# lmdu/pyfastx

Hardware: AMD Instinct MI355X
Metric: FASTA index build + 1M random 100bp subseq fetches, 3 Gbp plain FASTA per GPU (throughput of the whole step, stream resident in HBM) (higher is better)
Workload: dtype u8; 1 GPU; configs[1]: synthetic 3.0 Gbp hg38-shaped plain FASTA per GPU (200 contigs, 60-col LF, soft-masked, N runs), index build + 1000000 random 100 bp intervals (50% '-' strand); parallelism=one GPU, the whole stream resident in its HBM

## Files before the change

### pyfastx_amd/csrc/fx_kernels.hpp

```cpp
#pragma once
#include <hip/hip_runtime.h>
#include <stdint.h>

namespace fx {

constexpr int BLOCK = 256;
constexpr int UNROLL = 8;
constexpr int CHUNK = 16;
constexpr int TILE = BLOCK * CHUNK * UNROLL;

__device__ __forceinline__ uint32_t zero_bytes(uint32_t x) {
    return ~(((x & 0x7F7F7F7Fu) + 0x7F7F7F7Fu) | x | 0x7F7F7F7Fu);
}
__device__ __forceinline__ uint32_t flags4(uint32_t t) { return __builtin_amdgcn_udot4(t, 0x08040201u, 0u, false) >> 7; }
__device__ __forceinline__ uint32_t eq_mask16(const uint4 &v, uint32_t pat) {
    uint32_t lo = __builtin_amdgcn_udot4(zero_bytes(v.x ^ pat), 0x08040201u, 0u, false);
    lo = __builtin_amdgcn_udot4(zero_bytes(v.y ^ pat), 0x80402010u, lo, false);
    uint32_t hi = __builtin_amdgcn_udot4(zero_bytes(v.z ^ pat), 0x08040201u, 0u, false);
    hi = __builtin_amdgcn_udot4(zero_bytes(v.w ^ pat), 0x80402010u, hi, false);
    return (lo >> 7) | (hi << 1);
}

__device__ __forceinline__ uint4 load16(const uint8_t *__restrict__ data, int64_t p, int64_t n) {
    if (p + CHUNK <= n) return *reinterpret_cast<const uint4 *>(data + p);
// ... 337 lines not shown
            }
            rank += total;
        }
        if (ok) {
            int64_t got = rank - skip;
            got = got < 0 ? 0 : (got > take ? take : got);
            if ((fl & 2) && got < take && got > 0) {
                const int64_t delta = take - got;
                for (int64_t j0 = 0; j0 < got; j0 += G) {
                    const int64_t j = j0 + sub;
                    uint8_t c = 0;
                    if (j < got) c = out[delta + j];
                    if (j < got) out[j] = c;
                }
            }
            if (sub == 0 && q.out_len) q.out_len[i] = got;
        }
    }
}

template <int G, int NP, bool COAL = false>
__global__ __launch_bounds__(BLOCK) void k_fetch_lines(const uint8_t *__restrict__ data, int64_t gbase, int64_t n_bytes, FetchQ q, FastaTab tab,
                                                      int64_t nq, int flags_all, uint8_t *__restrict__ dst, int32_t *__restrict__ list,
                                                      int *__restrict__ list_n) {
    __shared__ uint8_t lut[256];
    constexpr int CO_CAP = 2048;
    __shared__ __attribute__((aligned(16))) uint32_t s_out[COAL ? BLOCK / 64 : 1][COAL ? (CO_CAP + 32) / 4 : 1];
    constexpr int TABCAP = 512;
    __shared__ int64_t s_boff[TABCAP], s_slen[TABCAP];
    __shared__ int32_t s_llen[TABCAP], s_en[TABCAP];
    const int64_t n_seq = tab.n_seq_dev ? (*tab.n_seq_dev < tab.n_seq ? (int64_t)*tab.n_seq_dev : tab.n_seq) : tab.n_seq;
    const bool tab_lds = n_seq <= TABCAP && n_seq > 0;
    build_comp_lut(lut);
    if (tab_lds)
        for (int r = threadIdx.x; r < (int)n_seq; r += BLOCK) {
            s_boff[r] = tab.boff[r]; s_slen[r] = tab.slen[r];
            const int64_t ll = tab.llen[r];
            s_llen[r] = ll > 0x7FFFFFFFll ? 0x7FFFFFFF : (int32_t)ll;
            s_en[r] = tab.elen[r] | (tab.norm[r] << 8);
        }
    __syncthreads();
    constexpr int QPW = 64 / G;
    const int lane = lane_id(), sub = lane & (G - 1), grp = lane / G;
    const int64_t wave = ((int64_t)blockIdx.x * BLOCK + threadIdx.x) >> 6;
    const int64_t nwaves = ((int64_t)gridDim.x * BLOCK) >> 6;
    int64_t d_id = 0, d_a = 0, d_b = 0, d_off = 0;
    int d_fl = flags_all;
    auto fetch_desc = [&](int64_t i) {
// ... 349 lines not shown
```

### pyfastx_amd/csrc/fx_spanscan.hpp

```cpp
#pragma once
#include "fx_kernels.hpp"

namespace fx {

#ifndef FX_GRAN
#define FX_GRAN 4096
#endif
constexpr int GRAN = FX_GRAN;
constexpr int GR_ROWS = GRAN / (64 * CHUNK);
constexpr int SPAN_GRANS = 65536 / GRAN;
constexpr int SPAN = GRAN * SPAN_GRANS;
constexpr uint32_t SP_NONE = 0xFFFFFFFFu;

struct GranOut { uint32_t n, h, first, last, v1, c1, v2, c2, ovf; };
struct __attribute__((aligned(16))) GranPk { uint32_t nh, fl, d1, d2; };
__device__ __forceinline__ GranPk gran_pack(const GranOut &o) {
    GranPk p;
    p.nh = o.n | (o.h << 16); p.fl = (o.first & 0xFFFFu) | (o.last << 16);
    p.d1 = o.v1 | (o.c1 << 16); p.d2 = o.v2 | (o.c2 << 16) | (o.ovf << 31);
    return p;
}
__device__ __forceinline__ GranOut gran_unpack(const GranPk &p) {
    GranOut o;
    o.n = p.nh & 0xFFFFu; o.h = p.nh >> 16;
// ... 206 lines not shown
    }
    const int64_t g0 = (((int64_t)blockIdx.x * blockDim.x + threadIdx.x) >> 6) * SCAN_GPW;
    uint4 v[SCAN_GPW][GR_ROWS];
#pragma unroll
    for (int k = 0; k < SCAN_GPW; ++k) if (g0 + k < g_end) granule_load<true>(v[k], data, n, is_last, g0 + k);
    uint32_t L = 0, hmask = 0;
#pragma unroll
    for (int k = 0; k < SCAN_GPW; ++k)
        if (g0 + k < g_end && granule_body<MODE>(v[k], data, prev_byte, g0 + k, out, L)) hmask |= 1u << k;
    if (MODE == 0 && lane_id() == 0) {
#pragma unroll
        for (int k = 0; k < SCAN_GPW; ++k) if ((hmask >> k) & 1u) hl_g[atomicAdd(&hl_n, 1u)] = (uint32_t)(g0 + k);
        __threadfence_block();
        if (atomicAdd(&hl_done, 1u) == (blockDim.x >> 6) - 1) {
            const uint32_t cnt = hl_n;
            if (cnt) {
                const uint32_t base = atomicAdd(hgl.count, cnt);
                for (uint32_t k = 0; k < cnt; ++k) hgl.g[base + k] = hl_g[k];
            }
        }
    }
}

constexpr int CHUNK_GRANS = 1024;
struct ChunkTot { long long n, h, last, pad; };
struct Totals {
    long long n_nl, n_hdr, last_nl, seq_len, pad0, pad1, pad2, pad3;
};

__device__ __forceinline__ long long shfl_up64(long long v, int d) {
    const int lo = __shfl_up((int)(v & 0xFFFFFFFFll), d, 64), hi = __shfl_up((int)(v >> 32), d, 64);
    return ((long long)hi << 32) | (unsigned int)lo;
}
__device__ __forceinline__ long long shfl64(long long v, int l) {
    const int lo = __shfl((int)(v & 0xFFFFFFFFll), l, 64), hi = __shfl((int)(v >> 32), l, 64);
    return ((long long)hi << 32) | (unsigned int)lo;
}
struct Tri { long long n, h, last; };
__device__ __forceinline__ Tri tri_join(const Tri &a, const Tri &b) { return Tri{a.n + b.n, a.h + b.h, a.last > b.last ? a.last : b.last}; }
__device__ __forceinline__ Tri tri_wave_incl(Tri v) {
    const int l = lane_id();
#pragma unroll
    for (int d = 1; d < 64; d <<= 1) {
        const Tri t{shfl_up64(v.n, d), shfl_up64(v.h, d), shfl_up64(v.last, d)};
        if (l >= d) v = tri_join(t, v);
    }
    return v;
}
__device__ __forceinline__ Tri tri_block_incl(Tri v, Tri *lds, Tri *total) {
    const int w = threadIdx.x >> 6, l = lane_id(), nw = (blockDim.x + 63) >> 6;
    const Tri inc = tri_wave_incl(v);
    __syncthreads();
    if (l == 63) lds[w] = inc;
    __syncthreads();
    Tri base{0, 0, -1}, tot{0, 0, -1};
    for (int i = 0; i < nw; ++i) { const Tri s = lds[i]; if (i < w) base = tri_join(base, s); tot = tri_join(tot, s); }
    *total = tot;
    return tri_join(base, inc);
}
__device__ __forceinline__ Tri gran_tri(const GranPk *__restrict__ go, int64_t g, int64_t ngran, int64_t gbase) {
    if (g >= ngran) return Tri{0, 0, -1};
    const GranOut o = gran_unpack(go[g]);
    return Tri{(long long)o.n, (long long)o.h, o.n ? gbase + g * (long long)GRAN + o.last : -1};
}

template <int MODE, int CG>
__global__ __launch_bounds__(CG) void k_gran_reduce(const uint8_t *__restrict__ data, int64_t n, int prev_byte,
                                                   int is_last, GranList hgl, GranPk *__restrict__ go,
                                                   int64_t ngran, int64_t gbase, ChunkTot *__restrict__ ct) {
    __shared__ Tri lds[CG / 64];
    if (blockIdx.x == gridDim.x - 1) {
        if (threadIdx.x < 64) {
            uint32_t L = 0;
            const uint32_t h_w = granule<false, MODE>(data, n, prev_byte, is_last, ngran - 1, go, L);
            if (MODE == 0 && h_w && threadIdx.x == 0) hgl.g[atomicAdd(hgl.count, 1u)] = (uint32_t)(ngran - 1);
        }
        __threadfence_block();
        __syncthreads();
    }
    Tri tot;
    tri_block_incl(gran_tri(go, (int64_t)blockIdx.x * CG + threadIdx.x, ngran, gbase), lds, &tot);
    if (threadIdx.x == 0) ct[blockIdx.x] = ChunkTot{tot.n, tot.h, tot.last, 0};
}

struct Tri32 { uint32_t n, h; int32_t last; };
__device__ __forceinline__ Tri32 tri32_block_incl(Tri32 v, uint32_t (*lds)[16], Tri32 *total) {
    const int w = threadIdx.x >> 6, l = lane_id(), nw = (blockDim.x + 63) >> 6;
#pragma unroll
    for (int d = 1; d < 64; d <<= 1) {
        const uint32_t a = __shfl_up(v.n, d, 64), b = __shfl_up(v.h, d, 64);
        const int32_t c = __shfl_up(v.last, d, 64);
        if (l >= d) { v.n += a; v.h += b; v.last = c > v.last ? c : v.last; }
    }
// ... 370 lines not shown
    const int64_t cnt = *irr.count;
    int64_t i = wave, g = i < cnt ? irr.g[i] : 0;
    uint4 v[GR_ROWS];
    if (i < cnt) {
#pragma unroll
        for (int j = 0; j < GR_ROWS; ++j) v[j] = load16(x.data, g * (int64_t)GRAN + j * 1024 + lane * CHUNK, x.n);
    }
    for (; i < cnt; i += nwaves) {
        const int64_t gc = g, hb = x.hdr_prefix[gc];
        int64_t he = x.hdr_prefix[gc + 1];
        if (he > cap) he = cap;
        ExactMasks mk;
        exact_masks(x, v, is_last, prev_byte, gc, he > hb, mk);
        if (i + nwaves < cnt) {
            g = irr.g[i + nwaves];
#pragma unroll
            for (int j = 0; j < GR_ROWS; ++j) v[j] = load16(x.data, g * (int64_t)GRAN + j * 1024 + lane * CHUNK, x.n);
        }
        exact_rows(x, rv, cap, gc, hb, mk);
    }
}

__global__ __launch_bounds__(BLOCK) void k_fasta_finalize2(int64_t cap, FastaCols c, Totals *__restrict__ tot,
                                                          const uint8_t *__restrict__ data, int64_t n_bytes, int64_t gbase) {
    const int64_t *__restrict__ hdr = c.hoff, *__restrict__ hdr_line = c.hdr_line;
    const int64_t k = (int64_t)blockIdx.x * BLOCK + threadIdx.x;
    const int64_t n_hdr = tot->n_hdr < cap ? tot->n_hdr : cap;
    int64_t s = 0;
    if (k < n_hdr) {
        if (c.dlen[k] >= 0) {
            int64_t hn, Ln;
            if (k + 1 < n_hdr) { hn = hdr[k + 1]; Ln = hdr_line[k + 1]; }
            else               { hn = tot->last_nl + 1; Ln = tot->n_nl; }
            const int64_t nseq = Ln - hdr_line[k] - 1;
            const int64_t blen = hn - c.boff[k];
            s = blen - (int64_t)c.elen[k] * nseq;
            c.blen[k] = blen; c.slen[k] = s;
            const int norm = c.bad[k] > 1 ? 0 : 1;
            c.norm[k] = norm;
            int reg = line_regular(data, n_bytes, gbase, c.boff[k], blen, s, nseq > 0 ? c.llen[k] : 0, c.elen[k], norm);
            if (reg < 0) reg = c.bad[k] == 0;
            c.reg[k] = reg;
        } else { c.blen[k] = 0; c.slen[k] = 0; c.norm[k] = 1; c.reg[k] = 0; }
    }
    __shared__ unsigned long long blk;
    if (threadIdx.x == 0) blk = 0;
    __syncthreads();
    s = wave_sum64(s);
    if (lane_id() == 0 && s) atomicAdd(&blk, (unsigned long long)s);
    __syncthreads();
    if (threadIdx.x == 0 && blk) atomicAdd((unsigned long long *)&tot->seq_len, blk);
}

__global__ __launch_bounds__(BLOCK) void k_line_regular(const uint8_t *__restrict__ data, int64_t n_bytes, int64_t gbase, int64_t n,
                                                       const int64_t *__restrict__ boff, const int64_t *__restrict__ blen,
                                                       const int64_t *__restrict__ slen, const int64_t *__restrict__ llen,
                                                       const int32_t *__restrict__ elen, const int32_t *__restrict__ norm,
                                                       int32_t *__restrict__ reg) {
    const int64_t k = (int64_t)blockIdx.x * BLOCK + threadIdx.x;
    if (k < n) reg[k] = line_regular(data, n_bytes, gbase, boff[k], blen[k], slen[k], llen[k], elen[k], norm[k]) > 0 ? 1 : 0;
}

__device__ __forceinline__ int64_t prev_nl_wave(const ScanCtx &x, int64_t p) {
    const int64_t y = (p - x.gbase < x.n) ? p - x.gbase : x.n;
    if (y <= 0) return -1;
    const int64_t g = (y - 1) / GRAN;
    const int64_t a = g * (int64_t)GRAN + lane_id() * 64;
    unsigned long long m = 0;
#pragma unroll
    for (int i = 0; i < 4; ++i)
        if (a + i * CHUNK < y) m |= (unsigned long long)eq_mask16(load16(x.data, a + i * CHUNK, x.n), 0x0A0A0A0Au) << (16 * i);
    if (y - a < 64) m &= (y - a <= 0) ? 0ull : (~0ull >> (64 - (y - a)));
    const unsigned long long b = __ballot(m != 0);
    if (!b) return x.prevnl[g];
// ... 220 lines not shown
```

### pyfastx_amd/csrc/fxgpu.hip

```cpp
#include <hip/hip_runtime.h>
#include <zlib.h>
#include <fcntl.h>
#include <pthread.h>
#include <sched.h>
#include <sys/mman.h>
#include <sys/stat.h>
#include <unistd.h>

#include <algorithm>
#include <atomic>
#include <chrono>
#include <functional>
#include <map>
#include <memory>
#include <cstdarg>
#include <cstdio>
#include <cstdlib>
#include <cstring>
#include <mutex>
#include <string>
#include <thread>
#include <vector>

#include "../../include/fxgpu.h"
// ... 307 lines not shown
static void stage_drop(fx_handle *h);
struct fx_handle {
    int device = 0;
    hipStream_t stream = nullptr;
    StageAsync *stage = nullptr;
    int stage_fd = -1;
    hipStream_t stream2 = nullptr;
    uint8_t *d_data = nullptr;
    uint8_t *d_alloc = nullptr;
    size_t blob_cap = 0;
    bool owns = false;
    int64_t n = 0;
    bool gz = false;
    int64_t base = 0;
    int prev_byte = '\n';
    bool is_last = true;
    int64_t n_nl = 0;
    bool scanned = false;
    int64_t ngran = 0;
    DevBuf<GranPk> gran;
    DevBuf<uint32_t> hdr_grans, irr_grans;
    DevBuf<ChunkTot> chunks;
    DevBuf<unsigned long long> ctl;
    Totals *pin_tot = nullptr;
    struct OneBox { int64_t off, blen, skip, take, dst_off, out_len; } *one_box = nullptr;
    uint8_t *one_out = nullptr;
    Mailbox *mb = nullptr;
    hipStream_t mb_stream = nullptr;
    unsigned long long mb_seq = 0;
    bool mb_running = false, mb_off = false;
    DevBuf<uint32_t> nm_table;
    DevBuf<int64_t> nm_off;
    uint64_t nm_mask = 0;
    int nm_kind = -1;
    DevBuf<int64_t> nl_prefix, hdr_prefix, prevnl;
    DevBuf<int64_t> hdr, fa_boff, fa_blen, fa_slen, fa_llen, fa_hdr_line;
    DevBuf<int32_t> fa_elen, fa_norm, fa_dlen, fa_name_len, fa_reg;
    DevBuf<uint32_t> fa_bad;
    int64_t n_hdr = 0, fa_seqlen = 0;
    bool fasta_built = false;
    bool build_pending = false;
    int pending_full_name = 0;
    DevBuf<uint32_t> comp_runs;
    int comp_gpw = 0;
    bool comp_runs_valid = false;
    DevBuf<int64_t> fq_name_off, fq_rlen, fq_soff, fq_qoff;
// ... 1538 lines not shown
static ScanCtx scan_ctx(const fx_handle *h) {
    ScanCtx x;
    x.data = h->d_data; x.n = h->n; x.gbase = h->base; x.ngran = h->ngran;
    x.go = h->gran.p; x.nl_prefix = h->nl_prefix.p; x.hdr_prefix = h->hdr_prefix.p; x.prevnl = h->prevnl.p;
    return x;
}
static FastaCols fasta_cols(fx_handle *h) {
    FastaCols c;
    c.hoff = h->hdr.p; c.boff = h->fa_boff.p; c.blen = h->fa_blen.p; c.slen = h->fa_slen.p; c.llen = h->fa_llen.p;
    c.hdr_line = h->fa_hdr_line.p; c.elen = h->fa_elen.p; c.dlen = h->fa_dlen.p; c.name_len = h->fa_name_len.p;
    c.norm = h->fa_norm.p; c.bad = h->fa_bad.p; c.reg = h->fa_reg.p;
    return c;
}
static int alloc_fasta_table(fx_handle *h, int64_t cap) {
    int rc;
    if ((rc = h->hdr.alloc(cap)) || (rc = h->fa_hdr_line.alloc(cap)) || (rc = h->fa_boff.alloc(cap)) ||
        (rc = h->fa_blen.alloc(cap)) || (rc = h->fa_slen.alloc(cap)) || (rc = h->fa_llen.alloc(cap)) ||
        (rc = h->fa_elen.alloc(cap)) || (rc = h->fa_norm.alloc(cap)) || (rc = h->fa_dlen.alloc(cap)) ||
        (rc = h->fa_name_len.alloc(cap)) || (rc = h->fa_bad.alloc(cap)) || (rc = h->fa_reg.alloc(cap)))
        return rc;
    return FX_OK;
}

static Totals *ctl_totals(fx_handle *h) { return (Totals *)h->ctl.p; }
static uint32_t *ctl_counter(fx_handle *h, int i) { return (uint32_t *)(h->ctl.p + 8 + i); }

static int comp_run_granules(int64_t ngran) {
    return ngran >= 65536 ? 4 * COMP_DEPTH : ngran >= 16384 ? 2 * COMP_DEPTH : COMP_DEPTH;
}

template <int MODE>
static int granule_pass(fx_handle *h, bool fq_lines = false, bool with_comp = false) {
    int rc;
    const int64_t nfull = h->n / GRAN, ngran = nfull + 1;
    const bool small = ngran <= (2ll << 20);
    const int64_t cg = small ? 256 : 1024, nchunks = (ngran + cg - 1) / cg;
    h->ngran = ngran;
    if ((rc = h->gran.alloc(ngran)) || (rc = h->hdr_grans.alloc(ngran)) || (MODE == 0 && (rc = h->irr_grans.alloc(ngran))) ||
        (rc = h->chunks.alloc(nchunks)) ||
        (rc = h->ctl.alloc(64)) || (rc = h->nl_prefix.alloc(ngran + 1)) || (rc = h->hdr_prefix.alloc(ngran + 1)) ||
        (rc = h->prevnl.alloc(ngran + 1)))
        return rc;
    if (!h->pin_tot) HIPCHK(hipHostMalloc((void **)&h->pin_tot, sizeof(Totals), hipHostMallocDefault));
    HIPCHK(hipMemsetAsync(h->ctl.p, 0, 64 * sizeof(unsigned long long), h->stream));
    GranList hgl{h->hdr_grans.p, ctl_counter(h, 0)};
    const int SCAN_WG = 512;
    if (nfull > 0 && MODE == 1 && fq_lines) {
        if ((rc = h->fq_lines.alloc((nfull + FQR_G - 1) / FQR_G * FQR_G * FQL_CAP))) return rc;
        if (with_comp) {
            const int64_t nruns = (nfull + FQLC_G - 1) / FQLC_G;
            if ((rc = h->fq_runs.alloc(nruns)) || (rc = h->fq_acc_build.alloc(1)) || (rc = h->fq_rej.alloc(nruns + 1))) return rc;
            static const int64_t grid_cap = [] { const char *e = getenv("FX_FQ_FUSED_GRID"); return e && atoll(e) > 0 ? atoll(e) : 6144ll; }();
            static const int force_crlf = [] { const char *e = getenv("FX_FQ_CRLF"); return e ? atoi(e) : -1; }();
            if (force_crlf >= 0 ? force_crlf != 0 : h->fq_crlf)
                FX_LAUNCH(h, K_FASTQ_LINES, k_fastq_lines_comp<true>, dim3((unsigned)std::min<int64_t>(nblocks(nruns, BLOCK / 64), grid_cap)), dim3(BLOCK), h->d_data,
                          h->n, h->prev_byte, nfull, h->gran.p, h->fq_lines.p, hgl, h->fq_runs.p, nruns);
            else
                FX_LAUNCH(h, K_FASTQ_LINES, k_fastq_lines_comp<false>, dim3((unsigned)std::min<int64_t>(nblocks(nruns, BLOCK / 64), grid_cap)), dim3(BLOCK), h->d_data,
                          h->n, h->prev_byte, nfull, h->gran.p, h->fq_lines.p, hgl, h->fq_runs.p, nruns);
        } else
        FX_LAUNCH(h, K_FASTQ_LINES, k_fastq_lines, dim3(nblocks(nfull, (BLOCK / 64) * FQL_G)), dim3(BLOCK), h->d_data, h->n, h->prev_byte, nfull,
                  h->gran.p, h->fq_lines.p, hgl);
    } else if (nfull > 0 && MODE == 0 && with_comp) {
        const int gpw = comp_run_granules(ngran);
        const int64_t runs = (ngran + gpw - 1) / gpw;
        if ((rc = h->comp_runs.alloc(runs * RUN_WORDS))) return rc;
        HIPCHK(hipMemsetAsync(h->comp_runs.p, 0, (size_t)runs * RUN_WORDS * 4, h->stream));
        FX_LAUNCH(h, K_SCAN_COMP, k_scan_comp, dim3(nblocks(runs, COMP_WPB)), dim3(COMP_WPB * 64), h->d_data, h->n, h->prev_byte,
                  (int)h->is_last, nfull, h->gran.p, hgl, gpw, h->comp_runs.p);
        h->comp_gpw = gpw;
        h->comp_runs_valid = true;
    } else if (nfull > 0)
        FX_LAUNCH(h, K_SPAN_SCAN, (k_span_scan<MODE>), dim3(nblocks((nfull + SCAN_GPW - 1) / SCAN_GPW * 64, SCAN_WG)), dim3(SCAN_WG), h->d_data, h->n,
                  h->prev_byte, (int)h->is_last, nfull, h->gran.p, hgl);
    if (small) {
        FX_LAUNCH(h, K_GRAN_REDUCE, (k_gran_reduce<MODE, 256>), dim3((unsigned)nchunks), dim3(256), h->d_data, h->n, h->prev_byte,
                  (int)h->is_last, hgl, h->gran.p, ngran, h->base, h->chunks.p);
        FX_LAUNCH(h, K_GRAN_PREFIX, (k_gran_prefix<256>), dim3((unsigned)nchunks), dim3(256), h->gran.p, ngran, h->base,
                  h->chunks.p, ctl_totals(h), h->nl_prefix.p, h->hdr_prefix.p, h->prevnl.p);
    } else {
        FX_LAUNCH(h, K_GRAN_REDUCE, (k_gran_reduce<MODE, 1024>), dim3((unsigned)nchunks), dim3(1024), h->d_data, h->n, h->prev_byte,
                  (int)h->is_last, hgl, h->gran.p, ngran, h->base, h->chunks.p);
        FX_LAUNCH(h, K_GRAN_PREFIX, (k_gran_prefix<1024>), dim3((unsigned)nchunks), dim3(1024), h->gran.p, ngran, h->base,
                  h->chunks.p, ctl_totals(h), h->nl_prefix.p, h->hdr_prefix.p, h->prevnl.p);
    }
    if (MODE == 1 && fq_lines && with_comp && nfull > 0) {
        FastqAcc init;
        memset(&init, 0, sizeof init);
        init.minqs = 104; init.maxqs = 33;
        HIPCHK(hipMemcpyAsync(h->fq_acc_build.p, &init, sizeof init, hipMemcpyHostToDevice, h->stream));
        const int64_t nruns = (nfull + FQLC_G - 1) / FQLC_G;
        HIPCHK(hipMemsetAsync(h->fq_rej.p, 0, 4, h->stream));
        FX_LAUNCH(h, K_FASTQ_COMP, k_fastq_comp_reduce, dim3((unsigned)std::min<int64_t>(nblocks(nruns, BLOCK), 1024)), dim3(BLOCK), (const FqRun *)h->fq_runs.p,
                  nruns, (const int64_t *)h->nl_prefix.p, (int64_t)0, h->d_data, h->n, nfull, h->fq_acc_build.p, h->fq_rej.p);
    }
    HIPCHK(hipGetLastError());
    return FX_OK;
}

static int enqueue_records(fx_handle *h, int full_name) {
    const ScanCtx x = scan_ctx(h);
    const int64_t cap = h->hdr.cap, ngran = h->ngran;
    const FastaCols c = fasta_cols(h);
    const RecView rv{h->fa_boff.p, h->fa_llen.p, h->fa_dlen.p, h->fa_bad.p, h->hdr.p};
    const GranList hgl{h->hdr_grans.p, ctl_counter(h, 0)}, irr{h->irr_grans.p, ctl_counter(h, 1)};
    FX_LAUNCH(h, K_HDR_REC, k_hdr_rec, dim3(2048), dim3(BLOCK), x, h->prev_byte, (int)h->is_last, full_name, hgl, c, cap);
    FX_LAUNCH(h, K_GRAN_LINES, k_gran_lines, dim3(nblocks(ngran, BLOCK)), dim3(BLOCK), x, rv, cap, irr);
    FX_LAUNCH(h, K_GRAN_EXACT, k_gran_exact, dim3(2048), dim3(BLOCK), x, rv, cap, irr, (int)h->is_last, h->prev_byte);
    FX_LAUNCH(h, K_FASTA_FINALIZE, k_fasta_finalize2, dim3(nblocks(cap, BLOCK)), dim3(BLOCK), cap, c, ctl_totals(h), h->d_data, h->n, h->base);
    HIPCHK(hipGetLastError());
    HIPCHK(hipMemcpyAsync(h->pin_tot, ctl_totals(h), sizeof(Totals), hipMemcpyDeviceToHost, h->stream));
    return FX_OK;
}

extern "C" int fx_fasta_build_begin(fx_handle *h, int full_name) {
    if (!h) return fail(FX_EINVAL, "null handle");
    int rc = use_device(h);
    if (rc) return rc;
    if (h->n <= 0) return fail(FX_EFORMAT, "empty input");
    h->scanned = false;
    h->nm_kind = -1;
    const bool with_comp = (full_name & 2) != 0;
    full_name &= 1;
    h->comp_runs_valid = false;
    if ((rc = granule_pass<0>(h, false, with_comp))) return rc;
    if (h->hdr.cap < 4096 && (rc = alloc_fasta_table(h, 4096))) return rc;
    if ((rc = enqueue_records(h, full_name))) return rc;
    h->build_pending = true;
    h->pending_full_name = full_name;
    h->fasta_built = true;
    return FX_OK;
}

static int finish_build(fx_handle *h) {
// ... 56 lines not shown

template <class T>
static int copy_out(fx_handle *h, int where, T *dst, const T *src, int64_t n) {
    if (!dst || n <= 0) return FX_OK;
    HIPCHK(hipMemcpyAsync(dst, src, (size_t)n * sizeof(T), where == FX_DEVICE ? hipMemcpyDeviceToDevice : hipMemcpyDeviceToHost, h->stream));
    return FX_OK;
}

extern "C" int fx_fasta_table(fx_handle *h, int where, int64_t *hoff, int64_t *boff, int64_t *blen, int64_t *slen,
                              int64_t *llen, int32_t *elen, int32_t *norm, int32_t *dlen, int32_t *name_len) {
    if (!h) return fail(FX_EINVAL, "null handle");
    if (!h->fasta_built) return fail(FX_ESTATE, "fx_fasta_build has not run");
    int rc = use_device(h);
    if (!rc) rc = finish_build(h);
    if (rc) return rc;
    const int64_t n = h->n_hdr;
    if ((rc = copy_out(h, where, hoff, h->hdr.p, n)) || (rc = copy_out(h, where, boff, h->fa_boff.p, n)) ||
        (rc = copy_out(h, where, blen, h->fa_blen.p, n)) || (rc = copy_out(h, where, slen, h->fa_slen.p, n)) ||
        (rc = copy_out(h, where, llen, h->fa_llen.p, n)) || (rc = copy_out(h, where, elen, h->fa_elen.p, n)) ||
        (rc = copy_out(h, where, norm, h->fa_norm.p, n)) || (rc = copy_out(h, where, dlen, h->fa_dlen.p, n)) ||
        (rc = copy_out(h, where, name_len, h->fa_name_len.p, n)))
        return rc;
    int stitch_err = 0;
    HIPCHK(hipMemcpyAsync(&stitch_err, h->ctl.p + 60, sizeof stitch_err, hipMemcpyDeviceToHost, h->stream));
    HIPCHK(hipStreamSynchronize(h->stream));
    if (stitch_err) return fail(FX_ERANGE, "header line crossing a shard cut continues for more than 64 KiB");
    return FX_OK;
}

static int fasta_comp_dense(fx_handle *h, int64_t lead_from, DevBuf<unsigned long long> &tmp, DevBuf<int32_t> &edge) {
    if (!h->fasta_built) return fail(FX_ESTATE, "fx_fasta_build has not run");
    int rc = use_device(h);
    if (!rc) rc = finish_build(h);
    if (rc) return rc;
    const int64_t n = h->n_hdr * 128;
    if ((rc = tmp.alloc(n + 128))) return rc;
    unsigned long long *d = tmp.p;
    HIPCHK(hipMemsetAsync(d, 0, (size_t)(n + 128) * 8, h->stream));
    const bool from_scan = h->comp_runs_valid;
    const int gpw = from_scan ? h->comp_gpw : comp_run_granules(h->ngran);
    const int64_t waves = (h->ngran + gpw - 1) / gpw;
    const dim3 grid((unsigned)((waves + COMP_WPB - 1) / COMP_WPB));
    if ((rc = edge.alloc(waves + 1))) return rc;
    HIPCHK(hipMemsetAsync(edge.p, 0, 4, h->stream));
    if (from_scan)
        FX_LAUNCH(h, K_COMP_ATTRIBUTE, k_comp_attribute, dim3(nblocks(waves, ATTR_BLOCK)), dim3(ATTR_BLOCK), h->comp_runs.p, waves, gpw, h->n,
                  h->base, h->fa_boff.p, h->n_hdr, h->hdr_prefix.p, h->ngran, lead_from, edge.p, d);
// ... 69 lines not shown
    HIPCHK(hipStreamSynchronize(h->stream));
    return FX_OK;
}

extern "C" int fx_fasta_comp(fx_handle *h, int where, int64_t *comp) { return fasta_comp_impl(h, where, comp, -1, nullptr); }

extern "C" int fx_fasta_comp_shard(fx_handle *h, int where, int64_t *comp, int64_t lead_from, int64_t *lead) {
    if (!lead) return fail(FX_EINVAL, "null argument");
    return fasta_comp_impl(h, where, comp, lead_from, lead);
}

static int fastq_count(fx_handle *h, int64_t *n_nl_core, int64_t *last_nl_core, bool want_comp = false) {
    int rc = use_device(h);
    if (rc) return rc;
    if (h->n <= 0) return fail(FX_EFORMAT, "empty input");
    h->fasta_built = h->fastq_built = h->comp_runs_valid = false;
    h->fq_comp_valid = false;
    static const int force = [] { const char *e = getenv("FX_FQ_LINES"); return e ? atoi(e) : -1; }();
    bool by_lines = force > 0;
    h->fq_crlf = false;
    memset(g_build_laps, 0, sizeof g_build_laps);
    LapClock lc;
    if (h->n >= 4 * GRAN) {
        if ((rc = h->ctl.alloc(64))) return rc;
        HIPCHK(hipMemsetAsync(h->ctl.p + 56, 0, 3 * sizeof(unsigned long long), h->stream));
        hipLaunchKernelGGL(k_nl_sample, dim3(3), dim3(BLOCK), 0, h->stream, h->d_data, h->n, h->ctl.p + 56);
        HIPCHK(hipGetLastError());
        unsigned long long smp[3];
        HIPCHK(hipMemcpyAsync(smp, h->ctl.p + 56, sizeof smp, hipMemcpyDeviceToHost, h->stream));
        HIPCHK(hipStreamSynchronize(h->stream));
        if (force < 0) by_lines = smp[1] > 0 && (double)smp[0] / (double)smp[1] * GRAN <= 0.7 * FQL_CAP;
        h->fq_crlf = smp[2] > 0;
    }
    static const bool no_fuse = [] { const char *e = getenv("FX_FQ_NO_FUSED_COMP"); return e && atoi(e) != 0; }();
    const bool with_comp = want_comp && by_lines && !no_fuse && h->base == 0 && h->halo == 0 && h->is_last && h->n >= GRAN;
    lc.lap(0);
    if ((rc = granule_pass<1>(h, by_lines, with_comp))) return rc;
    lc.lap(1);
    int64_t *res = (int64_t *)(h->ctl.p + 48);
    hipLaunchKernelGGL(k_core_count, dim3(1), dim3(64), 0, h->stream, scan_ctx(h), (int)h->is_last, h->n - h->halo, res);
    HIPCHK(hipGetLastError());
    int64_t host[3];
    HIPCHK(hipMemcpyAsync(h->pin_tot, ctl_totals(h), sizeof(Totals), hipMemcpyDeviceToHost, h->stream));
    HIPCHK(hipMemcpyAsync(host, res, sizeof host, hipMemcpyDeviceToHost, h->stream));
    uint32_t n_over = 0;
    if (by_lines) HIPCHK(hipMemcpyAsync(&n_over, ctl_counter(h, 0), sizeof n_over, hipMemcpyDeviceToHost, h->stream));
    FastqAcc built;
    memset(&built, 0, sizeof built);
    uint32_t n_rej = 0;
    if (with_comp) {
        HIPCHK(hipMemcpyAsync(&built, h->fq_acc_build.p, sizeof built, hipMemcpyDeviceToHost, h->stream));
        HIPCHK(hipMemcpyAsync(&n_rej, h->fq_rej.p, 4, hipMemcpyDeviceToHost, h->stream));
    }
    HIPCHK(hipStreamSynchronize(h->stream));
    lc.lap(2);
    if (with_comp) {
        const int64_t nfull = h->n / GRAN, nruns = (nfull + FQLC_G - 1) / FQLC_G;
        h->fq_comp_runs = nruns;
        h->fq_comp_rejected = n_rej;
        static const int64_t rej_div = [] { const char *e = getenv("FX_FQ_RECOUNT_DIV"); return e && atoll(e) > 0 ? atoll(e) : 8ll; }();
        if (built.qfix == 0 && n_rej > 0) {
            if ((int64_t)n_rej <= std::max<int64_t>(64, nruns / rej_div)) {
// ... 491 lines not shown
        *dst = (T *)d;
        return FX_OK;
    }
};

static unsigned fetch_grid(int64_t nq) {
    static const int64_t cap = []() { const char *e = getenv("FX_FETCH_WG"); const int64_t v = e ? atoll(e) : 0; return v > 0 ? v : (int64_t)256 * 8 * 4; }();
    return (unsigned)std::max<int64_t>(1, std::min<int64_t>((nq + 3) / 4, cap));
}

static int fetch_launch(fx_handle *h, Staged &st, const FetchQ &q, bool by_id, bool longq, int64_t n, int flags, uint8_t *d_dst) {
    int rc;
    FastaTab tab;
    memset(&tab, 0, sizeof tab);
    if (h->fasta_built) {
        tab.boff = h->fa_boff.p; tab.blen = h->fa_blen.p; tab.slen = h->fa_slen.p; tab.llen = h->fa_llen.p;
        tab.elen = h->fa_elen.p; tab.norm = h->fa_reg.p; tab.n_seq = h->n_hdr;
        if (h->build_pending) { tab.n_seq_dev = (const long long *)&ctl_totals(h)->n_hdr; tab.n_seq = h->hdr.cap; }
    }
    static const int fetch_g = [] { const char *e = getenv("FX_FETCH_G"); return e ? atoi(e) : 4; }();
    static const bool lean = [] { const char *e = getenv("FX_FETCH_LEAN"); return !e || atoi(e) != 0; }();
    if (!longq && by_id && fetch_g == 4 && lean && n < 0x7FFFFFFFll) {
        int32_t *d_list = nullptr;
        int *d_cnt = nullptr;
        if ((rc = st.scratch<int32_t>(n, &d_list)) || (rc = st.scratch<int>(1, &d_cnt))) return rc;
        HIPCHK(hipMemsetAsync(d_cnt, 0, sizeof(int), h->stream));
        static const int np = [] { const char *e = getenv("FX_FETCH_NP"); return e ? atoi(e) : 1; }();
        static const bool coal = [] { const char *e = getenv("FX_FETCH_COAL"); return e && atoi(e) != 0; }();
        if (np == 1 && coal) FX_LAUNCH(h, K_FETCH, (k_fetch_lines<4, 1, true>), dim3(fetch_grid((n + 15) / 16)), dim3(BLOCK), h->d_data, h->base, h->n, q, tab, n, flags, d_dst, d_list, d_cnt);
        else if (np == 1) FX_LAUNCH(h, K_FETCH, (k_fetch_lines<4, 1>), dim3(fetch_grid((n + 15) / 16)), dim3(BLOCK), h->d_data, h->base, h->n, q, tab, n, flags, d_dst, d_list, d_cnt);
        else         FX_LAUNCH(h, K_FETCH, (k_fetch_lines<4, 2>), dim3(fetch_grid((n + 15) / 16)), dim3(BLOCK), h->d_data, h->base, h->n, q, tab, n, flags, d_dst, d_list, d_cnt);
        FX_LAUNCH(h, K_FETCH_REST, (k_fetch<true, 4, 16>), dim3(std::min(fetch_grid((n + 15) / 16), 1024u)), dim3(BLOCK), h->d_data, h->base, h->n, q, tab, n, flags,
                  d_dst, (const int32_t *)d_list, (const int *)d_cnt);
    } else if (!longq && by_id && fetch_g == 4) {
        FX_LAUNCH(h, K_FETCH, (k_fetch<true, 4, 16>), dim3(fetch_grid((n + 15) / 16)), dim3(BLOCK), h->d_data, h->base, h->n, q, tab, n, flags, d_dst);
    } else if (!longq && by_id && fetch_g == 2) {
        FX_LAUNCH(h, K_FETCH, (k_fetch<true, 2, 16>), dim3(fetch_grid((n + 31) / 32)), dim3(BLOCK), h->d_data, h->base, h->n, q, tab, n, flags, d_dst);
    } else if (!longq && by_id && fetch_g == 16) {
        FX_LAUNCH(h, K_FETCH, (k_fetch<true, 16, 16>), dim3(fetch_grid((n + 3) / 4)), dim3(BLOCK), h->d_data, h->base, h->n, q, tab, n, flags, d_dst);
    } else if (!longq) {
        const unsigned grid8 = fetch_grid((n + 7) / 8);
        if (by_id) FX_LAUNCH(h, K_FETCH, (k_fetch<true, 8, 16>), dim3(grid8), dim3(BLOCK), h->d_data, h->base, h->n, q, tab, n, flags, d_dst);
        else       FX_LAUNCH(h, K_FETCH, (k_fetch<false, 8, 16>), dim3(grid8), dim3(BLOCK), h->d_data, h->base, h->n, q, tab, n, flags, d_dst);
    } else {
        const unsigned grid = fetch_grid(n);
        if (by_id) FX_LAUNCH(h, K_FETCH, (k_fetch<true, 64, 16>), dim3(grid), dim3(BLOCK), h->d_data, h->base, h->n, q, tab, n, flags, d_dst);
        else       FX_LAUNCH(h, K_FETCH, (k_fetch<false, 64, 16>), dim3(grid), dim3(BLOCK), h->d_data, h->base, h->n, q, tab, n, flags, d_dst);
    }
    HIPCHK(hipGetLastError());
    return FX_OK;
}

static int fetch_common(fx_handle *h, int where, int64_t n, bool by_id, const int64_t *a0, const int64_t *a1,
                        const int64_t *a2, const int64_t *skip, int flags, const uint8_t *qflags, uint8_t *dst,
                        const int64_t *dst_off, int64_t *out_len, int64_t dst_bytes_hint) {
    if (!h) return fail(FX_EINVAL, "null handle");
// ... 1354 lines not shown

extern "C" int fx_prof_read(fx_handle *h, int id, double *total_ms, int64_t *launches) {
    if (!h || id < 0 || id >= K_NKERN) return fail(FX_EINVAL, "bad argument");
    int rc = fx_sync(h);
    if (rc) return rc;
    if (total_ms) *total_ms = h->prof.ms[id];
    if (launches) *launches = h->prof.cnt[id];
    return FX_OK;
}

static int shard_summary_launch(fx_handle *h, int64_t *d_out) {
    static_assert(sizeof(fx_shard_summary) == SS_WORDS * 8, "summary layout");
    if (!h->fasta_built) return fail(FX_ESTATE, "fx_fasta_build has not run");
    int rc = use_device(h);
    if (rc) return rc;
    hipLaunchKernelGGL(k_shard_summary2, dim3(1), dim3(SUMM_BLOCK), 0, h->stream, scan_ctx(h), (int)h->is_last, ctl_totals(h),
                       h->hdr.cap, h->hdr.p, h->fa_hdr_line.p, fasta_cols(h), d_out);
    HIPCHK(hipGetLastError());
    return FX_OK;
}

extern "C" int fx_shard_summary_get(fx_handle *h, fx_shard_summary *out) {
    if (!h || !out) return fail(FX_EINVAL, "null argument");
    int64_t *S = h->ctl.p ? (int64_t *)(h->ctl.p + 16) : nullptr;
    int rc = shard_summary_launch(h, S);
    if (rc) return rc;
    HIPCHK(hipMemcpyAsync(out, S, sizeof(fx_shard_summary), hipMemcpyDeviceToHost, h->stream));
    HIPCHK(hipStreamSynchronize(h->stream));
    return FX_OK;
}

extern "C" int fx_shard_summary_dev(fx_handle *h, int64_t *d_out) {
    if (!h || !d_out) return fail(FX_EINVAL, "null argument");
    return shard_summary_launch(h, d_out);
}

extern "C" int fx_fasta_stitch_dev(fx_handle *h, const int64_t *d_all, int world, int rank, int full_name) {
    if (!h || !d_all || world < 1 || rank < 0 || rank >= world) return fail(FX_EINVAL, "bad argument");
    if (!h->fasta_built) return fail(FX_ESTATE, "fx_fasta_build has not run");
    int rc = use_device(h);
    if (!rc) rc = finish_build(h);
    if (rc) return rc;
    hipLaunchKernelGGL(k_stitch_tail, dim3(1), dim3(1), 0, h->stream, d_all, world, rank, full_name, fasta_cols(h), h->hdr.cap,
                       (int *)(h->ctl.p + 60));
    HIPCHK(hipGetLastError());
    return FX_OK;
}

extern "C" void *fx_stream(fx_handle *h) { return h ? (void *)h->stream : nullptr; }

extern "C" int fx_fasta_line_regular(fx_handle *h, int where, int32_t *reg) {
    if (!h || !reg) return fail(FX_EINVAL, "null argument");
    if (!h->fasta_built) return fail(FX_ESTATE, "fx_fasta_build has not run");
    int rc = use_device(h);
    if (!rc) rc = finish_build(h);
    if (rc) return rc;
    if ((rc = copy_out(h, where, reg, h->fa_reg.p, h->n_hdr))) return rc;
    HIPCHK(hipStreamSynchronize(h->stream));
    return FX_OK;
}

extern "C" int fx_fasta_set_row(fx_handle *h, int64_t k, int64_t boff, int64_t blen, int64_t slen, int64_t llen,
                                int32_t elen, int32_t norm, int32_t dlen, int32_t name_len) {
    if (!h) return fail(FX_EINVAL, "null handle");
    if (!h->fasta_built) return fail(FX_ESTATE, "fx_fasta_build has not run");
    int rc = use_device(h);
    if (!rc) rc = finish_build(h);
// ... 1069 lines not shown
```

Before: 4886 Gbp/s.

## Double-buffer control words and counters to drop per-call memsets and D2H copy

The control block and the fetch list counter each get a second bank that alternates between calls. The kernel running in the current call zeroes the other bank, so the next call can skip its hipMemsetAsync. The finalize kernel also gains a last-block ticket that writes the totals straight into pinned host memory, replacing a separate D2H memcpy when the header count is small. This removes several tiny stream operations and their launch latency, in exchange for more state tracking on the handle and an ordering hazard if a call aborts between the bank switch and the cleanup.

Result: no change. 4875 Gbp/s (-0.2%).

```diff
diff --git a/pyfastx_amd/csrc/fx_kernels.hpp b/pyfastx_amd/csrc/fx_kernels.hpp
--- a/pyfastx_amd/csrc/fx_kernels.hpp
+++ b/pyfastx_amd/csrc/fx_kernels.hpp
@@ -383,8 +383,9 @@
 template <int G, int NP, bool COAL = false>
 __global__ __launch_bounds__(BLOCK) void k_fetch_lines(const uint8_t *__restrict__ data, int64_t gbase, int64_t n_bytes, FetchQ q, FastaTab tab,
                                                       int64_t nq, int flags_all, uint8_t *__restrict__ dst, int32_t *__restrict__ list,
-                                                      int *__restrict__ list_n) {
+                                                      int *__restrict__ list_n, int *__restrict__ list_n_other) {
     __shared__ uint8_t lut[256];
+    if (blockIdx.x == 0 && threadIdx.x == 0 && list_n_other) *list_n_other = 0;
     constexpr int CO_CAP = 2048;
     __shared__ __attribute__((aligned(16))) uint32_t s_out[COAL ? BLOCK / 64 : 1][COAL ? (CO_CAP + 32) / 4 : 1];
     constexpr int TABCAP = 512;
diff --git a/pyfastx_amd/csrc/fx_spanscan.hpp b/pyfastx_amd/csrc/fx_spanscan.hpp
--- a/pyfastx_amd/csrc/fx_spanscan.hpp
+++ b/pyfastx_amd/csrc/fx_spanscan.hpp
@@ -252,11 +252,14 @@
     }
 }
 
+constexpr int CTL_WORDS = 64;
 constexpr int CHUNK_GRANS = 1024;
 struct ChunkTot { long long n, h, last, pad; };
 struct Totals {
     long long n_nl, n_hdr, last_nl, seq_len, pad0, pad1, pad2, pad3;
 };
+
+static_assert(offsetof(Totals, seq_len) == 24 && sizeof(Totals) == 64, "k_fasta_finalize2 hands the eight words over, seq_len being word 3");
 
 __device__ __forceinline__ long long shfl_up64(long long v, int d) {
     const int lo = __shfl_up((int)(v & 0xFFFFFFFFll), d, 64), hi = __shfl_up((int)(v >> 32), d, 64);
@@ -297,8 +300,10 @@
 template <int MODE, int CG>
 __global__ __launch_bounds__(CG) void k_gran_reduce(const uint8_t *__restrict__ data, int64_t n, int prev_byte,
                                                    int is_last, GranList hgl, GranPk *__restrict__ go,
-                                                   int64_t ngran, int64_t gbase, ChunkTot *__restrict__ ct) {
+                                                   int64_t ngran, int64_t gbase, ChunkTot *__restrict__ ct,
+                                                   unsigned long long *__restrict__ ctl_other) {
     __shared__ Tri lds[CG / 64];
+    if (blockIdx.x == 0 && threadIdx.x < CTL_WORDS && ctl_other) ctl_other[threadIdx.x] = 0;
     if (blockIdx.x == gridDim.x - 1) {
         if (threadIdx.x < 64) {
             uint32_t L = 0;
@@ -715,7 +720,8 @@
 }
 
 __global__ __launch_bounds__(BLOCK) void k_fasta_finalize2(int64_t cap, FastaCols c, Totals *__restrict__ tot,
-                                                          const uint8_t *__restrict__ data, int64_t n_bytes, int64_t gbase) {
+                                                          const uint8_t *__restrict__ data, int64_t n_bytes, int64_t gbase,
+                                                          Totals *host_tot, uint32_t *ticket) {
     const int64_t *__restrict__ hdr = c.hoff, *__restrict__ hdr_line = c.hdr_line;
     const int64_t k = (int64_t)blockIdx.x * BLOCK + threadIdx.x;
     const int64_t n_hdr = tot->n_hdr < cap ? tot->n_hdr : cap;
@@ -743,6 +749,21 @@
     if (lane_id() == 0 && s) atomicAdd(&blk, (unsigned long long)s);
     __syncthreads();
     if (threadIdx.x == 0 && blk) atomicAdd((unsigned long long *)&tot->seq_len, blk);
+    if (!host_tot) return;
+    __shared__ uint32_t last;
+    if (threadIdx.x == 0) {
+        __threadfence();
+        last = atomicAdd(ticket, 1u) == gridDim.x - 1;
+    }
+    __syncthreads();
+    if (last && threadIdx.x < sizeof(Totals) / 8) {
+        __threadfence();
+        unsigned long long *src = (unsigned long long *)tot;
+        const unsigned long long v = threadIdx.x == 3 ? atomicAdd(&src[3], 0ull) : src[threadIdx.x];
+        ((volatile unsigned long long *)host_tot)[threadIdx.x] = v;
+        __threadfence_system();
+        if (threadIdx.x == 0) *ticket = 0;
+    }
 }
 
 __global__ __launch_bounds__(BLOCK) void k_line_regular(const uint8_t *__restrict__ data, int64_t n_bytes, int64_t gbase, int64_t n,
diff --git a/pyfastx_amd/csrc/fxgpu.hip b/pyfastx_amd/csrc/fxgpu.hip
--- a/pyfastx_amd/csrc/fxgpu.hip
+++ b/pyfastx_amd/csrc/fxgpu.hip
@@ -353,6 +353,11 @@
     DevBuf<uint32_t> hdr_grans, irr_grans;
     DevBuf<ChunkTot> chunks;
     DevBuf<unsigned long long> ctl;
+    int ctl_cur = 0;
+    DevBuf<int> fetch_cnt;
+    int fetch_cnt_cur = 0;
+    bool fetch_cnt_next_clean = false;
+    bool ctl_next_clean = false;
     Totals *pin_tot = nullptr;
     struct OneBox { int64_t off, blen, skip, take, dst_off, out_len; } *one_box = nullptr;
     uint8_t *one_out = nullptr;
@@ -1937,8 +1942,19 @@
     return FX_OK;
 }
 
-static Totals *ctl_totals(fx_handle *h) { return (Totals *)h->ctl.p; }
-static uint32_t *ctl_counter(fx_handle *h, int i) { return (uint32_t *)(h->ctl.p + 8 + i); }
+static unsigned long long *ctl_bank(fx_handle *h) { return h->ctl.p ? h->ctl.p + (size_t)h->ctl_cur * CTL_WORDS : nullptr; }
+static int ctl_alloc(fx_handle *h) {
+    if (h->ctl.p) return FX_OK;
+    int rc = h->ctl.alloc(2 * CTL_WORDS);
+    if (rc) return rc;
+    h->ctl_cur = 0;
+    h->ctl_next_clean = false;
+    HIPCHK(hipMemsetAsync(h->ctl.p, 0, 2 * CTL_WORDS * sizeof(unsigned long long), h->stream));
+    h->ctl_next_clean = true;
+    return FX_OK;
+}
+static Totals *ctl_totals(fx_handle *h) { return (Totals *)ctl_bank(h); }
+static uint32_t *ctl_counter(fx_handle *h, int i) { return (uint32_t *)(ctl_bank(h) + 8 + i); }
 
 static int comp_run_granules(int64_t ngran) {
     return ngran >= 65536 ? 4 * COMP_DEPTH : ngran >= 16384 ? 2 * COMP_DEPTH : COMP_DEPTH;
@@ -1953,11 +1969,14 @@
     h->ngran = ngran;
     if ((rc = h->gran.alloc(ngran)) || (rc = h->hdr_grans.alloc(ngran)) || (MODE == 0 && (rc = h->irr_grans.alloc(ngran))) ||
         (rc = h->chunks.alloc(nchunks)) ||
-        (rc = h->ctl.alloc(64)) || (rc = h->nl_prefix.alloc(ngran + 1)) || (rc = h->hdr_prefix.alloc(ngran + 1)) ||
+        (rc = ctl_alloc(h)) || (rc = h->nl_prefix.alloc(ngran + 1)) || (rc = h->hdr_prefix.alloc(ngran + 1)) ||
         (rc = h->prevnl.alloc(ngran + 1)))
         return rc;
     if (!h->pin_tot) HIPCHK(hipHostMalloc((void **)&h->pin_tot, sizeof(Totals), hipHostMallocDefault));
-    HIPCHK(hipMemsetAsync(h->ctl.p, 0, 64 * sizeof(unsigned long long), h->stream));
+    unsigned long long *const ctl_prev = ctl_bank(h);
+    h->ctl_cur ^= 1;
+    if (!h->ctl_next_clean) HIPCHK(hipMemsetAsync(ctl_bank(h), 0, CTL_WORDS * sizeof(unsigned long long), h->stream));
+    h->ctl_next_clean = false;
     GranList hgl{h->hdr_grans.p, ctl_counter(h, 0)};
     const int SCAN_WG = 512;
     if (nfull > 0 && MODE == 1 && fq_lines) {
@@ -1990,12 +2009,12 @@
                   h->prev_byte, (int)h->is_last, nfull, h->gran.p, hgl);
     if (small) {
         FX_LAUNCH(h, K_GRAN_REDUCE, (k_gran_reduce<MODE, 256>), dim3((unsigned)nchunks), dim3(256), h->d_data, h->n, h->prev_byte,
-                  (int)h->is_last, hgl, h->gran.p, ngran, h->base, h->chunks.p);
+                  (int)h->is_last, hgl, h->gran.p, ngran, h->base, h->chunks.p, ctl_prev);
         FX_LAUNCH(h, K_GRAN_PREFIX, (k_gran_prefix<256>), dim3((unsigned)nchunks), dim3(256), h->gran.p, ngran, h->base,
                   h->chunks.p, ctl_totals(h), h->nl_prefix.p, h->hdr_prefix.p, h->prevnl.p);
     } else {
         FX_LAUNCH(h, K_GRAN_REDUCE, (k_gran_reduce<MODE, 1024>), dim3((unsigned)nchunks), dim3(1024), h->d_data, h->n, h->prev_byte,
-                  (int)h->is_last, hgl, h->gran.p, ngran, h->base, h->chunks.p);
+                  (int)h->is_last, hgl, h->gran.p, ngran, h->base, h->chunks.p, ctl_prev);
         FX_LAUNCH(h, K_GRAN_PREFIX, (k_gran_prefix<1024>), dim3((unsigned)nchunks), dim3(1024), h->gran.p, ngran, h->base,
                   h->chunks.p, ctl_totals(h), h->nl_prefix.p, h->hdr_prefix.p, h->prevnl.p);
     }
@@ -2010,9 +2029,11 @@
                   nruns, (const int64_t *)h->nl_prefix.p, (int64_t)0, h->d_data, h->n, nfull, h->fq_acc_build.p, h->fq_rej.p);
     }
     HIPCHK(hipGetLastError());
-    return FX_OK;
-}
-
+    h->ctl_next_clean = true;
+    return FX_OK;
+}
+
+constexpr int64_t FINALIZE_TICKET_CAP = 65536;
 static int enqueue_records(fx_handle *h, int full_name) {
     const ScanCtx x = scan_ctx(h);
     const int64_t cap = h->hdr.cap, ngran = h->ngran;
@@ -2022,9 +2043,11 @@
     FX_LAUNCH(h, K_HDR_REC, k_hdr_rec, dim3(2048), dim3(BLOCK), x, h->prev_byte, (int)h->is_last, full_name, hgl, c, cap);
     FX_LAUNCH(h, K_GRAN_LINES, k_gran_lines, dim3(nblocks(ngran, BLOCK)), dim3(BLOCK), x, rv, cap, irr);
     FX_LAUNCH(h, K_GRAN_EXACT, k_gran_exact, dim3(2048), dim3(BLOCK), x, rv, cap, irr, (int)h->is_last, h->prev_byte);
-    FX_LAUNCH(h, K_FASTA_FINALIZE, k_fasta_finalize2, dim3(nblocks(cap, BLOCK)), dim3(BLOCK), cap, c, ctl_totals(h), h->d_data, h->n, h->base);
+    const bool by_ticket = cap <= FINALIZE_TICKET_CAP;
+    FX_LAUNCH(h, K_FASTA_FINALIZE, k_fasta_finalize2, dim3(nblocks(cap, BLOCK)), dim3(BLOCK), cap, c, ctl_totals(h), h->d_data, h->n, h->base,
+              by_ticket ? h->pin_tot : (Totals *)nullptr, ctl_counter(h, 2));
     HIPCHK(hipGetLastError());
-    HIPCHK(hipMemcpyAsync(h->pin_tot, ctl_totals(h), sizeof(Totals), hipMemcpyDeviceToHost, h->stream));
+    if (!by_ticket) HIPCHK(hipMemcpyAsync(h->pin_tot, ctl_totals(h), sizeof(Totals), hipMemcpyDeviceToHost, h->stream));
     return FX_OK;
 }
 
@@ -2127,7 +2150,7 @@
         (rc = copy_out(h, where, name_len, h->fa_name_len.p, n)))
         return rc;
     int stitch_err = 0;
-    HIPCHK(hipMemcpyAsync(&stitch_err, h->ctl.p + 60, sizeof stitch_err, hipMemcpyDeviceToHost, h->stream));
+    HIPCHK(hipMemcpyAsync(&stitch_err, ctl_bank(h) + 60, sizeof stitch_err, hipMemcpyDeviceToHost, h->stream));
     HIPCHK(hipStreamSynchronize(h->stream));
     if (stitch_err) return fail(FX_ERANGE, "header line crossing a shard cut continues for more than 64 KiB");
     return FX_OK;
@@ -2243,12 +2266,12 @@
     memset(g_build_laps, 0, sizeof g_build_laps);
     LapClock lc;
     if (h->n >= 4 * GRAN) {
-        if ((rc = h->ctl.alloc(64))) return rc;
-        HIPCHK(hipMemsetAsync(h->ctl.p + 56, 0, 3 * sizeof(unsigned long long), h->stream));
-        hipLaunchKernelGGL(k_nl_sample, dim3(3), dim3(BLOCK), 0, h->stream, h->d_data, h->n, h->ctl.p + 56);
+        if ((rc = ctl_alloc(h))) return rc;
+        HIPCHK(hipMemsetAsync(ctl_bank(h) + 56, 0, 3 * sizeof(unsigned long long), h->stream));
+        hipLaunchKernelGGL(k_nl_sample, dim3(3), dim3(BLOCK), 0, h->stream, h->d_data, h->n, ctl_bank(h) + 56);
         HIPCHK(hipGetLastError());
         unsigned long long smp[3];
-        HIPCHK(hipMemcpyAsync(smp, h->ctl.p + 56, sizeof smp, hipMemcpyDeviceToHost, h->stream));
+        HIPCHK(hipMemcpyAsync(smp, ctl_bank(h) + 56, sizeof smp, hipMemcpyDeviceToHost, h->stream));
         HIPCHK(hipStreamSynchronize(h->stream));
         if (force < 0) by_lines = smp[1] > 0 && (double)smp[0] / (double)smp[1] * GRAN <= 0.7 * FQL_CAP;
         h->fq_crlf = smp[2] > 0;
@@ -2258,7 +2281,7 @@
     lc.lap(0);
     if ((rc = granule_pass<1>(h, by_lines, with_comp))) return rc;
     lc.lap(1);
-    int64_t *res = (int64_t *)(h->ctl.p + 48);
+    int64_t *res = (int64_t *)(ctl_bank(h) + 48);
     hipLaunchKernelGGL(k_core_count, dim3(1), dim3(64), 0, h->stream, scan_ctx(h), (int)h->is_last, h->n - h->halo, res);
     HIPCHK(hipGetLastError());
     int64_t host[3];
@@ -2796,16 +2819,27 @@
     static const bool lean = [] { const char *e = getenv("FX_FETCH_LEAN"); return !e || atoi(e) != 0; }();
     if (!longq && by_id && fetch_g == 4 && lean && n < 0x7FFFFFFFll) {
         int32_t *d_list = nullptr;
-        int *d_cnt = nullptr;
-        if ((rc = st.scratch<int32_t>(n, &d_list)) || (rc = st.scratch<int>(1, &d_cnt))) return rc;
-        HIPCHK(hipMemsetAsync(d_cnt, 0, sizeof(int), h->stream));
+        if ((rc = st.scratch<int32_t>(n, &d_list))) return rc;
+        if (!h->fetch_cnt.p) {
+            if ((rc = h->fetch_cnt.alloc(2))) return rc;
+            HIPCHK(hipMemsetAsync(h->fetch_cnt.p, 0, 2 * sizeof(int), h->stream));
+            h->fetch_cnt_cur = 0;
+            h->fetch_cnt_next_clean = true;
+        }
+        int *const d_cnt_other = h->fetch_cnt.p + h->fetch_cnt_cur;
+        h->fetch_cnt_cur ^= 1;
+        int *const d_cnt = h->fetch_cnt.p + h->fetch_cnt_cur;
+        if (!h->fetch_cnt_next_clean) HIPCHK(hipMemsetAsync(d_cnt, 0, sizeof(int), h->stream));
+        h->fetch_cnt_next_clean = false;
         static const int np = [] { const char *e = getenv("FX_FETCH_NP"); return e ? atoi(e) : 1; }();
         static const bool coal = [] { const char *e = getenv("FX_FETCH_COAL"); return e && atoi(e) != 0; }();
-        if (np == 1 && coal) FX_LAUNCH(h, K_FETCH, (k_fetch_lines<4, 1, true>), dim3(fetch_grid((n + 15) / 16)), dim3(BLOCK), h->d_data, h->base, h->n, q, tab, n, flags, d_dst, d_list, d_cnt);
-        else if (np == 1) FX_LAUNCH(h, K_FETCH, (k_fetch_lines<4, 1>), dim3(fetch_grid((n + 15) / 16)), dim3(BLOCK), h->d_data, h->base, h->n, q, tab, n, flags, d_dst, d_list, d_cnt);
-        else         FX_LAUNCH(h, K_FETCH, (k_fetch_lines<4, 2>), dim3(fetch_grid((n + 15) / 16)), dim3(BLOCK), h->d_data, h->base, h->n, q, tab, n, flags, d_dst, d_list, d_cnt);
+        if (np == 1 && coal) FX_LAUNCH(h, K_FETCH, (k_fetch_lines<4, 1, true>), dim3(fetch_grid((n + 15) / 16)), dim3(BLOCK), h->d_data, h->base, h->n, q, tab, n, flags, d_dst, d_list, d_cnt, d_cnt_other);
+        else if (np == 1) FX_LAUNCH(h, K_FETCH, (k_fetch_lines<4, 1>), dim3(fetch_grid((n + 15) / 16)), dim3(BLOCK), h->d_data, h->base, h->n, q, tab, n, flags, d_dst, d_list, d_cnt, d_cnt_other);
+        else         FX_LAUNCH(h, K_FETCH, (k_fetch_lines<4, 2>), dim3(fetch_grid((n + 15) / 16)), dim3(BLOCK), h->d_data, h->base, h->n, q, tab, n, flags, d_dst, d_list, d_cnt, d_cnt_other);
         FX_LAUNCH(h, K_FETCH_REST, (k_fetch<true, 4, 16>), dim3(std::min(fetch_grid((n + 15) / 16), 1024u)), dim3(BLOCK), h->d_data, h->base, h->n, q, tab, n, flags,
                   d_dst, (const int32_t *)d_list, (const int *)d_cnt);
+        HIPCHK(hipGetLastError());
+        h->fetch_cnt_next_clean = true;
     } else if (!longq && by_id && fetch_g == 4) {
         FX_LAUNCH(h, K_FETCH, (k_fetch<true, 4, 16>), dim3(fetch_grid((n + 15) / 16)), dim3(BLOCK), h->d_data, h->base, h->n, q, tab, n, flags, d_dst);
     } else if (!longq && by_id && fetch_g == 2) {
@@ -4206,7 +4240,7 @@
 
 extern "C" int fx_shard_summary_get(fx_handle *h, fx_shard_summary *out) {
     if (!h || !out) return fail(FX_EINVAL, "null argument");
-    int64_t *S = h->ctl.p ? (int64_t *)(h->ctl.p + 16) : nullptr;
+    int64_t *S = h->ctl.p ? (int64_t *)(ctl_bank(h) + 16) : nullptr;
     int rc = shard_summary_launch(h, S);
     if (rc) return rc;
     HIPCHK(hipMemcpyAsync(out, S, sizeof(fx_shard_summary), hipMemcpyDeviceToHost, h->stream));
@@ -4226,7 +4260,7 @@
     if (!rc) rc = finish_build(h);
     if (rc) return rc;
     hipLaunchKernelGGL(k_stitch_tail, dim3(1), dim3(1), 0, h->stream, d_all, world, rank, full_name, fasta_cols(h), h->hdr.cap,
-                       (int *)(h->ctl.p + 60));
+                       (int *)(ctl_bank(h) + 60));
     HIPCHK(hipGetLastError());
     return FX_OK;
 }
```
